# GestaltCogTeam/STEP

Hardware: AMD Instinct MI355X
Metric: training windows/sec on PEMS04, horizon-12 MAE parity, 1/2/4/8 MI355X (higher is better)
Workload: dtype f16 (TSFormer Q/K/weights) + bf16 (P, V, GraphWaveNet / graph-learner GEMMs) operands, f32 accumulate

## Files before the change

step_amd/csrc/common.h:

```cpp
#pragma once
#include "../../include/step_hip.h"
#include <hip/hip_runtime.h>
#include <stdint.h>
#include <stdio.h>
#include <string.h>

#define STEP_OK 0
#define STEP_ERR_ARG 1
#define STEP_ERR_HIP 2

void step_set_error(const char* fmt, ...);
int step_raise_lds_once(const void* kernel, int bytes, const char* what);

#define STEP_REQUIRE(cond, ...)                 \
    do {                                        \
        if (!(cond)) {                          \
            step_set_error(__VA_ARGS__);        \
            return STEP_ERR_ARG;                \
        }                                       \
    } while (0)

#define STEP_LAUNCH_CHECK(name)                                                   \
    do {                                                                          \
        hipError_t e_ = hipGetLastError();                                        \
        if (e_ != hipSuccess) {                                                   \
            step_set_error("%s: launch failed: %s", name, hipGetErrorString(e_)); \
            return STEP_ERR_HIP;                                                  \
        }                                                                         \
    } while (0)

#define STEP_TRY(expr)                       \
    do {                                     \
        int rc_ = (expr);                    \
        if (rc_ != STEP_OK) return rc_;      \
    } while (0)

typedef __attribute__((ext_vector_type(16))) float f32x16;
typedef __attribute__((ext_vector_type(4))) float f32x4;
typedef __attribute__((ext_vector_type(8))) __bf16 bf16x8;
typedef __attribute__((ext_vector_type(4))) uint32_t u32x4;
typedef __attribute__((ext_vector_type(2))) uint32_t u32x2;

static inline int cdiv(long a, long b) { return (int)((a + b - 1) / b); }

__device__ __forceinline__ uint32_t f32_to_bf16_bits(float f) {
    uint32_t u = __float_as_uint(f);
    u += 0x7fffu + ((u >> 16) & 1u);
    return u >> 16;
}
__device__ __forceinline__ uint32_t pack_bf16x2(float lo, float hi) {
    return f32_to_bf16_bits(lo) | (f32_to_bf16_bits(hi) << 16);
}
__device__ __forceinline__ float bf16_bits_to_f32(uint32_t b) { return __uint_as_float(b << 16); }

typedef __attribute__((ext_vector_type(8))) float f32x8;
__device__ __forceinline__ bf16x8 pack8(const float* v) {
    f32x8 t;
#pragma unroll
    for (int j = 0; j < 8; ++j) t[j] = v[j];
    return __builtin_convertvector(t, bf16x8);
}

__device__ __forceinline__ float wave_sum(float v) {
#pragma unroll
    for (int o = 32; o > 0; o >>= 1) v += __shfl_xor(v, o, 64);
    return v;
}
__device__ __forceinline__ float wave_max(float v) {
#pragma unroll
    for (int o = 32; o > 0; o >>= 1) v = fmaxf(v, __shfl_xor(v, o, 64));
    return v;
}

#ifndef STEP_PHILOX_MUL64
#define STEP_PHILOX_MUL64 1
#endif
__device__ __forceinline__ void philox4x32(uint32_t c0, uint32_t c1, uint32_t c2, uint32_t c3,
                                           uint32_t k0, uint32_t k1, uint32_t out[4]) {
#pragma unroll
    for (int r = 0; r < 10; ++r) {
#if STEP_PHILOX_MUL64
        const uint64_t p0 = (uint64_t)0xD2511F53u * c0, p1 = (uint64_t)0xCD9E8D57u * c2;
        const uint32_t hi0 = (uint32_t)(p0 >> 32), lo0 = (uint32_t)p0, hi1 = (uint32_t)(p1 >> 32), lo1 = (uint32_t)p1;
#else
        uint32_t hi0 = __umulhi(0xD2511F53u, c0), lo0 = 0xD2511F53u * c0;
        uint32_t hi1 = __umulhi(0xCD9E8D57u, c2), lo1 = 0xCD9E8D57u * c2;
#endif
        uint32_t n0 = hi1 ^ c1 ^ k0, n1 = lo1, n2 = hi0 ^ c3 ^ k1, n3 = lo0;
        c0 = n0; c1 = n1; c2 = n2; c3 = n3;
        k0 += 0x9E3779B9u; k1 += 0xBB67AE85u;
    }
    out[0] = c0; out[1] = c1; out[2] = c2; out[3] = c3;
}
__device__ __forceinline__ float u32_to_unit(uint32_t x) { return (float)(x >> 8) * (1.0f / 16777216.0f); }

struct GemmColAffine { float cs, csh; const float* mvec; };
__device__ __forceinline__ GemmColAffine gemm_col_affine(const StepGemm& g, int gn) {
    GemmColAffine a = {1.f, 0.f, nullptr};
    if (g.c_nscale) { const int c = gn / g.c_nperiod; a.cs = g.c_nscale[c]; a.csh = g.c_nshift[c]; a.mvec = g.c_mvec; }
    return a;
}

__device__ __forceinline__ void gemm_store_tile(const f32x16& acc, float* col, int mb, int M, long ldc, float alpha, int accumulate,
                                                float bv, int relu, GemmColAffine ca = GemmColAffine{1.f, 0.f, nullptr}) {
    float val[16];
#pragma unroll
    for (int e = 0; e < 16; ++e) {
        const int gm = mb + (e & 3) + 8 * (e >> 2);
        val[e] = alpha * acc[e] * ca.cs;
        if (ca.mvec) val[e] += ca.csh * (gm < M ? ca.mvec[gm] : 0.f);
    }
    if (accumulate == 2) {
#pragma unroll
        for (int e = 0; e < 16; ++e) {
            const int gm = mb + (e & 3) + 8 * (e >> 2);
            if (gm < M) atomicAdd(col + (long)gm * ldc, val[e]);
        }
    } else if (accumulate == 1) {
        float old[16];
// ... 23 lines not shown
```

step_amd/csrc/dgl.hip:

```cpp
#include "common.h"
#include "step_internal.h"

namespace {

constexpr int KW = 10;
constexpr int EMB = 100;

template <int CI, int CO, int TPT>
__global__ __launch_bounds__(256) void conv_relu_fwd_kernel(const float* __restrict__ in, const float* __restrict__ w,
                                                            const float* __restrict__ b, const float* __restrict__ in_sc,
                                                            const float* __restrict__ in_sh, float* __restrict__ out,
                                                            float* __restrict__ partial, int Tin, int stat_limit) {
    __shared__ __attribute__((aligned(16))) float ws[CI * KW * CO];
    __shared__ float red[4][2 * CO];
    const int tid = threadIdx.x, n = blockIdx.y;
    const int Tout = Tin - (KW - 1);
    for (int e = tid; e < CI * KW * CO; e += 256) {
        int co = e % CO, k = (e / CO) % KW, ci = e / (CO * KW);
        ws[e] = w[(co * CI + ci) * KW + k];
    }
    __syncthreads();
    const int t0 = (blockIdx.x * 256 + tid) * TPT;
    float acc[CO][TPT];
#pragma unroll
// ... 412 lines not shown
                                                            const StepDynState* __restrict__ dyn) {
    if (dyn) { const uint64_t x = dyn->seed_xor; seed_lo ^= (uint32_t)x; seed_hi ^= (uint32_t)(x >> 32); }
    const long E = (long)N * N;
    const int b = blockIdx.y;
    for (long e = (long)blockIdx.x * 256 + threadIdx.x; e < E; e += (long)gridDim.x * 256) {
        const float zv = z[e];
        float u0, u1;
        if (u) {
            u0 = u[((long)b * E + e) * 2];
            u1 = u[((long)b * E + e) * 2 + 1];
        } else {
            uint32_t r[4];
            philox4x32((uint32_t)e, (uint32_t)(e >> 32), (uint32_t)b, 0x5EEDu, seed_lo, seed_hi, r);
            u0 = u32_to_unit(r[0]); u1 = u32_to_unit(r[1]);
        }
        const float g0 = -logf(-logf(u0 + 1e-10f) + 1e-10f);
        const float g1 = -logf(-logf(u1 + 1e-10f) + 1e-10f);
        const float a0 = (zv + g0 - g1) * inv_tau;
        const float ys = 1.f / (1.f + __expf(-a0));
        const int i = (int)(e / N), j = (int)(e % N);
        theta[(long)b * E + e] = 1.f / (1.f + __expf(-zv));
        y0[(long)b * E + e] = ys;
        adj[(long)b * E + e] = (i != j && a0 >= 0.f) ? 1.f : 0.f;
    }
}

__global__ __launch_bounds__(256) void edge_dz_kernel(const float* __restrict__ dtheta, const float* __restrict__ dadj,
                                                      const float* __restrict__ theta, const float* __restrict__ y0, int B, int N,
                                                      float inv_tau, float* __restrict__ dz) {
    const long E = (long)N * N;
    for (long e = (long)blockIdx.x * 256 + threadIdx.x; e < E; e += (long)gridDim.x * 256) {
        const int i = (int)(e / N), j = (int)(e % N);
        float s = 0.f;
        for (int b = 0; b < B; ++b) {
            const long o = (long)b * E + e;
            float th = theta[o];
            if (dtheta) s += dtheta[o] * th * (1.f - th);
            if (dadj && i != j) { float y = y0[o]; s += dadj[o] * y * (1.f - y) * inv_tau; }
        }
        dz[e] = s;
    }
}

__global__ __launch_bounds__(256) void edge_bwd_row_kernel(const float* __restrict__ dz, const float* __restrict__ sndT,
                                                           const float* __restrict__ rcv, const float* __restrict__ wcat, int N,
                                                           float* __restrict__ drcv, float* __restrict__ dwcat, float* __restrict__ dbcat) {
    extern __shared__ float sdz[];
    __shared__ float sr[EMB], sw[EMB], ra[EMB], rh[EMB];
    __shared__ float red[4];
    const int i = blockIdx.x, tid = threadIdx.x, lane = tid & 63, wave = tid >> 6;
    if (tid < EMB) { sr[tid] = rcv[(long)i * EMB + tid]; sw[tid] = wcat[tid] - wcat[EMB + tid]; }
    float tot = 0.f;
    for (int j = tid; j < N; j += 256) { const float d = dz[(long)i * N + j]; sdz[j] = d; tot += d; }
    tot = wave_sum(tot);
    if (lane == 0) red[wave] = tot;
    __syncthreads();
    constexpr int FB = 5;
    static_assert(EMB % (4 * FB) == 0, "feature rounds");
    for (int f0 = wave * FB; f0 < EMB; f0 += 4 * FB) {
        float a[FB], h[FB], rf[FB];
        const float* srow[FB];
#pragma unroll
        for (int u = 0; u < FB; ++u) { a[u] = 0.f; h[u] = 0.f; rf[u] = sr[f0 + u]; srow[u] = sndT + (long)(f0 + u) * N; }
        const bool vec = (N & 3) == 0 && ((((uintptr_t)sndT) | ((uintptr_t)sdz)) & 15) == 0;
        const int n4 = vec ? N : 0;
        for (int j = 4 * lane; j < n4; j += 256) {
            const float4 d4 = *(const float4*)(sdz + j);
            float4 s4[FB];
#pragma unroll
            for (int u = 0; u < FB; ++u) s4[u] = *(const float4*)(srow[u] + j);
#pragma unroll
            for (int u = 0; u < FB; ++u) {
                const float h0 = rf[u] + s4[u].x, h1 = rf[u] + s4[u].y, h2 = rf[u] + s4[u].z, h3 = rf[u] + s4[u].w;
                const float m0 = h0 > 0.f ? d4.x : 0.f, m1 = h1 > 0.f ? d4.y : 0.f, m2 = h2 > 0.f ? d4.z : 0.f, m3 = h3 > 0.f ? d4.w : 0.f;
                a[u] += (m0 + m1) + (m2 + m3);
                h[u] += (m0 * h0 + m1 * h1) + (m2 * h2 + m3 * h3);
            }
        }
        for (int j = n4 + lane; j < N; j += 64) {
            const float d = sdz[j];
            float sv[FB];
#pragma unroll
            for (int u = 0; u < FB; ++u) sv[u] = srow[u][j];
#pragma unroll
            for (int u = 0; u < FB; ++u) {
                const float hid = rf[u] + sv[u];
                const float m = hid > 0.f ? d : 0.f;
                a[u] += m; h[u] += m * hid;
            }
        }
#pragma unroll
        for (int o = 32; o > 0; o >>= 1)
#pragma unroll
            for (int u = 0; u < FB; ++u) { a[u] += __shfl_xor(a[u], o, 64); h[u] += __shfl_xor(h[u], o, 64); }
        if (lane == 0) {
#pragma unroll
            for (int u = 0; u < FB; ++u) { ra[f0 + u] = a[u]; rh[f0 + u] = h[u]; }
        }
    }
    __syncthreads();
    if (tid < EMB) {
        drcv[(long)i * EMB + tid] = ra[tid] * sw[tid];
        atomicAdd(&dwcat[tid], rh[tid]);
        atomicAdd(&dwcat[EMB + tid], -rh[tid]);
    }
    if (tid == 0) {
        const float s = red[0] + red[1] + red[2] + red[3];
        atomicAdd(&dbcat[0], s);
        atomicAdd(&dbcat[1], -s);
    }
}
template <int VJ>
__global__ __launch_bounds__(256) void edge_bwd_col_kernel(const float* __restrict__ dz, const float* __restrict__ sndT,
                                                           const float* __restrict__ rcv, const float* __restrict__ wcat, int N,
                                                           float* __restrict__ dsndT) {
    const int lane = threadIdx.x & 63, wave = threadIdx.x >> 6;
    const int j = (blockIdx.x * 64 + lane) * VJ;
    const int f = blockIdx.y * 4 + wave;
    if (j >= N || f >= EMB) return;
    const float wd = wcat[f] - wcat[EMB + f];
    if constexpr (VJ == 4) {
        const float4 s4 = *(const float4*)(sndT + (long)f * N + j);
        float a0 = 0.f, a1 = 0.f, a2 = 0.f, a3 = 0.f;
#pragma unroll 8
        for (int i = 0; i < N; ++i) {
            const float r = rcv[(long)i * EMB + f];
            const float4 d = *(const float4*)(dz + (long)i * N + j);
            a0 += r + s4.x > 0.f ? d.x : 0.f; a1 += r + s4.y > 0.f ? d.y : 0.f;
            a2 += r + s4.z > 0.f ? d.z : 0.f; a3 += r + s4.w > 0.f ? d.w : 0.f;
        }
        *(float4*)(dsndT + (long)f * N + j) = make_float4(a0 * wd, a1 * wd, a2 * wd, a3 * wd);
    } else {
        const float s = sndT[(long)f * N + j];
        float a = 0.f;
#pragma unroll 8
        for (int i = 0; i < N; ++i) {
            float hid = rcv[(long)i * EMB + f] + s;
            float d = dz[(long)i * N + j];
            a += hid > 0.f ? d : 0.f;
        }
        dsndT[(long)f * N + j] = a * wd;
    }
}

__global__ void colsum_kernel(const float* __restrict__ x, long rows, int cols, long ld, float* __restrict__ out) {
    __shared__ float red[4][64];
    const int c = blockIdx.x * 64 + (threadIdx.x & 63);
// ... 10 lines not shown

int step_colsum_launch(const float* x, long rows, int cols, long ld, float* out, hipStream_t st) {
    int chunks = (int)((rows + 255) / 256);
    if (chunks > 512) chunks = 512;
    if (chunks < 1) chunks = 1;
    colsum_kernel<<<dim3(cdiv(cols, 64), chunks), 256, 0, st>>>(x, rows, cols, ld, out);
    STEP_LAUNCH_CHECK("colsum");
    return STEP_OK;
}

constexpr int DGL_SMALL = 256 + 64 + 1344 + 100 * 32;

__global__ void bn2_fused_coef_kernel(const float* __restrict__ dots, const float* __restrict__ stat, const float* __restrict__ gamma,
                                      double count, float* __restrict__ dgamma, float* __restrict__ dbeta, float* __restrict__ coef) {
    constexpr int C = 16;
    const int c = threadIdx.x;
    if (c >= C) return;
    const float S1 = dots[2 * c + 1];
    const float S2 = stat[3 * C + c] * (dots[2 * c] - stat[2 * C + c] * S1);
    dgamma[c] += S2;
    dbeta[c] += S1;
    coef[c] = (float)(S1 / count);
    coef[C + c] = (float)(S2 / count);
    coef[2 * C + c] = gamma[c] * stat[3 * C + c];
}

__global__ __launch_bounds__(256) void fc_prep_kernel(const float* __restrict__ fc_w, const float* __restrict__ st2, uint4* __restrict__ wp,
                                                      float* __restrict__ shiftdot, int T2) {
    __shared__ float red[4];
    const int o = blockIdx.y, t = blockIdx.x * 256 + threadIdx.x, tid = threadIdx.x;
    float acc = 0.f;
    if (t < T2) {
        float v[16];
#pragma unroll
        for (int c = 0; c < 16; ++c) v[c] = fc_w[((long)o * 16 + c) * T2 + t];
#pragma unroll
        for (int c = 0; c < 16; ++c) { acc += v[c] * st2[16 + c]; v[c] *= st2[c]; }
        uint4* dst = wp + ((long)o * T2 + t) * 2;
        dst[0] = make_uint4(pack_bf16x2(v[0], v[1]), pack_bf16x2(v[2], v[3]), pack_bf16x2(v[4], v[5]), pack_bf16x2(v[6], v[7]));
        dst[1] = make_uint4(pack_bf16x2(v[8], v[9]), pack_bf16x2(v[10], v[11]), pack_bf16x2(v[12], v[13]), pack_bf16x2(v[14], v[15]));
    }
    acc = wave_sum(acc);
    if ((tid & 63) == 0) red[tid >> 6] = acc;
    __syncthreads();
    if (tid == 0) atomicAdd(&shiftdot[o], red[0] + red[1] + red[2] + red[3]);
}
__global__ void gpre_init_kernel(float* __restrict__ gpre, const float* __restrict__ shiftdot, long n) {
    const long i = (long)blockIdx.x * 256 + threadIdx.x;
    if (i < n) gpre[i] = shiftdot[i % EMB];
}
__global__ __launch_bounds__(256) void fc_unpermute_kernel(const float* __restrict__ graw, const float* __restrict__ fc_w,
                                                           const float* __restrict__ st2, const float* __restrict__ colsum,
                                                           float* __restrict__ dfc_w, float* __restrict__ dots_o, int T2, int overwrite) {
    __shared__ float red[4][32];
    const int o = blockIdx.y, t = blockIdx.x * 256 + threadIdx.x, tid = threadIdx.x;
    const float cso = colsum[o];
    float d[32];
#pragma unroll
    for (int i = 0; i < 32; ++i) d[i] = 0.f;
    if (t < T2) {
        const float4* src = (const float4*)(graw + ((long)o * T2 + t) * 16);
        const float4 g0 = src[0], g1 = src[1], g2 = src[2], g3 = src[3];
        const float g[16] = {g0.x, g0.y, g0.z, g0.w, g1.x, g1.y, g1.z, g1.w, g2.x, g2.y, g2.z, g2.w, g3.x, g3.y, g3.z, g3.w};
        float w[16], old[16];
#pragma unroll
        for (int c = 0; c < 16; ++c) { const long idx = ((long)o * 16 + c) * T2 + t; w[c] = fc_w[idx]; old[c] = overwrite ? 0.f : dfc_w[idx]; }
#pragma unroll
        for (int c = 0; c < 16; ++c) {
            dfc_w[((long)o * 16 + c) * T2 + t] = old[c] + st2[c] * g[c] + st2[16 + c] * cso;
            d[2 * c] = w[c] * g[c]; d[2 * c + 1] = w[c] * cso;
        }
    }
#pragma unroll
    for (int i = 0; i < 32; ++i) {
        const float v = wave_sum(d[i]);
        if ((tid & 63) == 0) red[tid >> 6][i] = v;
    }
    __syncthreads();
    if (tid < 32) atomicAdd(&dots_o[o * 32 + tid], red[0][tid] + red[1][tid] + red[2][tid] + red[3][tid]);
}
__global__ void dots_reduce_kernel(const float* __restrict__ dots_o, float* __restrict__ dots) {
    const int i = threadIdx.x;
    if (i >= 32) return;
    double a = 0.0;
    for (int o = 0; o < EMB; ++o) a += dots_o[o * 32 + i];
    dots[i] = (float)a;
}

static bool dgl_channels_last(const StepDglParams* p) {
    const char* e = getenv("STEP_DGL_F32_STORAGE");
    return p->gemm_bf16 && !(e && e[0] == '1');
}

static bool dgl_legacy_bn_backward() {
    const char* e = getenv("STEP_DGL_LEGACY_BN");
    return e && e[0] == '1';
}

extern "C" long step_dgl_global_saved_floats(int N, int T) {
    long T1 = T - 9, T2 = T - 18;
    return (long)N * 8 * T1 + (long)N * 16 * T2 + (long)N * EMB + 4 * 8 + 4 * 16 + 4 * EMB + (long)EMB * 16 * T2 + 128;
}
static long fc_splitk_ws_floats(int N, int T2) {
    const int splits = step_gemm_auto_splitk(N, EMB, 16 * T2, 1);
    return splits > 1 ? (long)splits * N * EMB + 4 : 0;
}
static long wraw_floats(long T2) {
    const long w = (long)EMB * 16 * T2, pack = dgl_conv2_pack_floats();
    return w > pack ? w : pack;
}
extern "C" long step_dgl_global_work_floats(int N, int T, int backward) {
    long T1 = T - 9, T2 = T - 18;
    long nb1 = (long)N * cdiv(T1, 1024), nb2 = (long)N * cdiv(T2, 1024);
    long part = (nb1 > nb2 ? nb1 : nb2) * 32 + 64;
    if (!backward) return part + dgl_conv2_pack_floats() + 64 + fc_splitk_ws_floats(N, (int)T2);
    return part + (long)N * 16 * T2 + (long)N * 8 * T1 + wraw_floats(T2) + 2L * N * EMB + DGL_SMALL + dgl_conv2_wgrad_scratch_floats(N, (int)T1);
}

static float* saved_wp(float* saved, int N, int T) {
    long T1 = T - 9, T2 = T - 18;
    return saved + (long)N * 8 * T1 + (long)N * 16 * T2 + (long)N * EMB + 4 * 8 + 4 * 16 + 4 * EMB;
}
static void carve_saved(float* saved, int N, int T, float** a1, float** a2, float** gpre, float** st1, float** st2, float** st3) {
    long T1 = T - 9, T2 = T - 18;
    *a1 = saved; saved += (long)N * 8 * T1;
    *a2 = saved; saved += (long)N * 16 * T2;
    *gpre = saved; saved += (long)N * EMB;
    *st1 = saved; saved += 4 * 8;
    *st2 = saved; saved += 4 * 16;
    *st3 = saved;
}

// ... 360 lines not shown
```

step_amd/csrc/dgl_conv_mfma.hip:

```cpp
#include "common.h"
#include "step_internal.h"

namespace {

constexpr int KW = 10, CI = 8, CO = 16, C1_ = 8;
constexpr int FW_TT = 1024;

__device__ __forceinline__ uint32_t cvt2(float a, float b) {
    uint32_t r;
    asm("v_cvt_pk_bf16_f32 %0, %1, %2" : "=v"(r) : "v"(a), "v"(b));
    return r;
}
__device__ __forceinline__ bf16x8 as_frag(uint4 v) { return __builtin_bit_cast(bf16x8, v); }

__global__ __launch_bounds__(256) void conv2_fwd_mfma_kernel(const float* __restrict__ a1, const float* __restrict__ w,
                                                             const float* __restrict__ b, const float* __restrict__ sc,
                                                             const float* __restrict__ sh, float* __restrict__ a2,
                                                             float* __restrict__ partial, int T1) {
    __shared__ uint4 xs[FW_TT + 16];
    __shared__ float red[4][2 * CO];
    const int tid = threadIdx.x, lane = tid & 63, wave = tid >> 6, n = blockIdx.y;
    const int T2 = T1 - (KW - 1), t0 = blockIdx.x * FW_TT;
    const int ln = lane & 15, q = lane >> 4;

// ... 315 lines not shown
#pragma unroll
            for (int co = 0; co < C1; ++co) {
                bsum[co] += v[co];
                zs[co][tid] = (uint16_t)(cvt2(v[co], 0.f) & 0xffffu);
            }
            const uint16_t ha = (uint16_t)(cvt2(xa, 0.f) & 0xffffu);
            x0[tid] = ha;
            if (tid > 0) x1[tid - 1] = ha;
            if (tid < 10) {
                const uint16_t hb = (uint16_t)(cvt2(xb, 0.f) & 0xffffu);
                x0[tid + 256] = hb;
                x1[tid + 255] = hb;
            }
        }
        __syncthreads();
        if (pass + 1 < WG_PASSES && tp + WG_SC < T1) fetch(tp + WG_SC);
#pragma unroll
        for (int u = 0; u < 2; ++u) {
            const int tb = 64 * wave + 32 * u + 8 * q;
            uint4 av = *(const uint4*)&zs[ln & 7][tb];
            if (ln >= C1) av = make_uint4(0u, 0u, 0u, 0u);
            const int kk = ln < KW ? ln : 0;
            const uint16_t* row = (kk & 1) ? x1 : x0;
            const uint32_t* p = (const uint32_t*)(row + tb + (kk & ~1));
            uint4 bv = make_uint4(p[0], p[1], p[2], p[3]);
            if (ln >= KW) bv = make_uint4(0u, 0u, 0u, 0u);
            acc = __builtin_amdgcn_mfma_f32_16x16x32_bf16(as_frag(av), as_frag(bv), acc, 0, 0, 0);
        }
    }
    __syncthreads();
    if (wave > 0) {
#pragma unroll
        for (int e = 0; e < 4; ++e) red[wave - 1][lane][e] = acc[e];
    }
#pragma unroll
    for (int co = 0; co < C1; ++co) {
        const float sm = wave_sum(bsum[co]);
        if (lane == 0) redb[wave][co] = sm;
    }
    __syncthreads();
    float* out = partial + ((long)blockIdx.y * gridDim.x + blockIdx.x) * W1_OUT;
    if (wave == 0 && q < 2 && ln < KW) {
#pragma unroll
        for (int e = 0; e < 4; ++e)
            out[(4 * q + e) * KW + ln] = acc[e] + red[0][lane][e] + red[1][lane][e] + red[2][lane][e];
    }
    if (tid < C1) out[C1 * KW + tid] = redb[0][tid] + redb[1][tid] + redb[2][tid] + redb[3][tid];
}


__device__ __forceinline__ float bf16lo(uint32_t w) { return __uint_as_float(w << 16); }
__device__ __forceinline__ float bf16hi(uint32_t w) { return __uint_as_float(w & 0xffff0000u); }

__global__ __launch_bounds__(256) void conv1_fwd_cl_kernel(const float* __restrict__ x, const float* __restrict__ w,
                                                           const float* __restrict__ b, uint4* __restrict__ a1h,
                                                           float* __restrict__ partial, int T, int stat_limit) {
    __shared__ float ws[KW][C1_];
    __shared__ float red[4][2 * C1_];
    __shared__ __attribute__((aligned(16))) float xs[1024 + 16];
    const int tid = threadIdx.x, n = blockIdx.y, T1 = T - (KW - 1);
    if (tid < KW * C1_) ws[tid / C1_][tid % C1_] = w[(tid % C1_) * KW + tid / C1_];
    {
        const int tb = blockIdx.x * 1024;
        const float* xr = x + (long)n * T + tb;
        for (int i = tid; i < 1024 + 16; i += 256) xs[i] = tb + i < T ? xr[i] : 0.f;
    }
    __syncthreads();
    const int t0 = (blockIdx.x * 256 + tid) * 4;
    float s1[C1_], s2[C1_];
#pragma unroll
    for (int c = 0; c < C1_; ++c) { s1[c] = 0.f; s2[c] = 0.f; }
    if (t0 < T1) {
        float xv[16];
#pragma unroll
        for (int q4 = 0; q4 < 4; ++q4) {
            const float4 v4 = *(const float4*)(xs + 4 * tid + 4 * q4);
            xv[4 * q4] = v4.x; xv[4 * q4 + 1] = v4.y; xv[4 * q4 + 2] = v4.z; xv[4 * q4 + 3] = v4.w;
        }
        float acc[4][C1_];
#pragma unroll
        for (int j = 0; j < 4; ++j)
#pragma unroll
            for (int c = 0; c < C1_; ++c) acc[j][c] = b[c];
#pragma unroll
        for (int k = 0; k < KW; ++k)
#pragma unroll
            for (int c = 0; c < C1_; ++c) {
                const float wv = ws[k][c];
#pragma unroll
                for (int j = 0; j < 4; ++j) acc[j][c] += wv * xv[k + j];
            }
#pragma unroll
        for (int j = 0; j < 4; ++j) {
            if (t0 + j >= T1) break;
            float v[C1_];
#pragma unroll
            for (int c = 0; c < C1_; ++c) {
                v[c] = fmaxf(acc[j][c], 0.f);
                if (t0 + j < stat_limit) { s1[c] += v[c]; s2[c] += v[c] * v[c]; }
            }
            a1h[(long)n * T1 + t0 + j] = make_uint4(cvt2(v[0], v[1]), cvt2(v[2], v[3]), cvt2(v[4], v[5]), cvt2(v[6], v[7]));
        }
    }
    const int lane = tid & 63, wave = tid >> 6;
#pragma unroll
    for (int c = 0; c < C1_; ++c) {
        const float a = wave_sum(s1[c]), q = wave_sum(s2[c]);
        if (lane == 0) { red[wave][c] = a; red[wave][C1_ + c] = q; }
    }
    __syncthreads();
    if (tid < 2 * C1_)
        partial[((long)blockIdx.y * gridDim.x + blockIdx.x) * (2 * C1_) + tid] = red[0][tid] + red[1][tid] + red[2][tid] + red[3][tid];
}

__global__ void conv2_pack_kernel(const float* __restrict__ w, const float* __restrict__ b, const float* __restrict__ sc,
                                  const float* __restrict__ sh, uint4* __restrict__ pack) {
    const int lane = threadIdx.x & 63, s = threadIdx.x >> 6, ln = lane & 15, q = lane >> 4;
    float v[8];
    if (s < 3) {
        const int kk = 4 * s + q;
#pragma unroll
        for (int ci = 0; ci < CI; ++ci) v[ci] = kk < KW ? w[(ln * CI + ci) * KW + kk] * sc[ci] : 0.f;
    } else {
        const int kk = 2 * (s - 3) + (q >> 1), c0 = 8 * (q & 1);
#pragma unroll
        for (int j = 0; j < 8; ++j) v[j] = ln < CI ? w[((c0 + j) * CI + ln) * KW + kk] * sc[ln] : 0.f;
    }
    pack[s * 64 + lane] = make_uint4(cvt2(v[0], v[1]), cvt2(v[2], v[3]), cvt2(v[4], v[5]), cvt2(v[6], v[7]));
    if (threadIdx.x < CO) {
        float a = b[threadIdx.x];
        for (int ci = 0; ci < CI; ++ci) {
            float ws = 0.f;
            for (int kk = 0; kk < KW; ++kk) ws += w[(threadIdx.x * CI + ci) * KW + kk];
            a += ws * sh[ci];
        }
        ((float*)(pack + 8 * 64))[threadIdx.x] = a;
    }
}

__global__ __launch_bounds__(256) void conv2_fwd_cl_kernel(const uint4* __restrict__ a1h, const uint4* __restrict__ pack,
                                                           uint2* __restrict__ a2h, float* __restrict__ partial, int T1) {
    __shared__ uint4 xs[FW_TT + 16];
    __shared__ float red[4][2 * CO];
    const int tid = threadIdx.x, lane = tid & 63, wave = tid >> 6, n = blockIdx.y;
    const int T2 = T1 - (KW - 1), t0 = blockIdx.x * FW_TT;
    const int ln = lane & 15, q = lane >> 4;
    for (int tt = tid; tt < FW_TT + 16; tt += 256) {
        const int t = t0 + tt;
        xs[tt] = t < T1 ? a1h[(long)n * T1 + t] : make_uint4(0u, 0u, 0u, 0u);
    }
    bf16x8 wf[3];
#pragma unroll
    for (int s = 0; s < 3; ++s) wf[s] = as_frag(pack[s * 64 + lane]);
    float bias[4];
#pragma unroll
    for (int e = 0; e < 4; ++e) bias[e] = ((const float*)(pack + 8 * 64))[4 * q + e];
    __syncthreads();
    float s1[4] = {0.f, 0.f, 0.f, 0.f}, s2[4] = {0.f, 0.f, 0.f, 0.f};
    for (int tile = wave; tile < FW_TT / 16; tile += 4) {
        const int tb = tile * 16;
        if (t0 + tb >= T2) break;
        f32x4 acc = {0.f, 0.f, 0.f, 0.f};
#pragma unroll
        for (int s = 0; s < 3; ++s) acc = __builtin_amdgcn_mfma_f32_16x16x32_bf16(wf[s], as_frag(xs[tb + ln + 4 * s + q]), acc, 0, 0, 0);
        const int t = t0 + tb + ln;
        if (t < T2) {
            float v[4];
#pragma unroll
            for (int e = 0; e < 4; ++e) { v[e] = fmaxf(acc[e] + bias[e], 0.f); s1[e] += v[e]; s2[e] += v[e] * v[e]; }
            a2h[((long)n * T2 + t) * 4 + q] = make_uint2(cvt2(v[0], v[1]), cvt2(v[2], v[3]));
        }
    }
#pragma unroll
    for (int e = 0; e < 4; ++e) {
#pragma unroll
        for (int o = 1; o < 16; o <<= 1) { s1[e] += __shfl_xor(s1[e], o, 64); s2[e] += __shfl_xor(s2[e], o, 64); }
        if (ln == 0) { red[wave][4 * q + e] = s1[e]; red[wave][CO + 4 * q + e] = s2[e]; }
    }
    __syncthreads();
    if (tid < 2 * CO)
        partial[((long)blockIdx.y * gridDim.x + blockIdx.x) * (2 * CO) + tid] = red[0][tid] + red[1][tid] + red[2][tid] + red[3][tid];
}

__global__ __launch_bounds__(256) void conv2_dgrad_cl_kernel(const uint4* __restrict__ dz2h, const uint4* __restrict__ pack,
                                                             uint2* __restrict__ dz1h, int T1,
                                                             const uint2* __restrict__ a1h, const float* __restrict__ coef,
                                                             const float* __restrict__ stat, int own) {
    __shared__ uint4 zs[FW_TT + 16][2];
    const int tid = threadIdx.x, lane = tid & 63, wave = tid >> 6, n = blockIdx.y;
    const int T2 = T1 - (KW - 1), t0 = blockIdx.x * FW_TT;
    const int ln = lane & 15, q = lane >> 4;
    constexpr int NT = FW_TT / 16 / 4;
    uint2 xall[NT];
    if (q < 2) {
#pragma unroll
        for (int i = 0; i < NT; ++i) {
            const int t = t0 + (wave + 4 * i) * 16 + ln;
            xall[i] = t < T1 ? a1h[((long)n * T1 + t) * 2 + q] : make_uint2(0u, 0u);
        }
    }
    for (int tt = tid; tt < FW_TT + 16; tt += 256) {
        const int t = t0 - (KW - 1) + tt;
        const bool ok = t >= 0 && t < T2;
        zs[tt][0] = ok ? dz2h[((long)n * T2 + t) * 2] : make_uint4(0u, 0u, 0u, 0u);
        zs[tt][1] = ok ? dz2h[((long)n * T2 + t) * 2 + 1] : make_uint4(0u, 0u, 0u, 0u);
    }
    bf16x8 wf[5];
#pragma unroll
    for (int s = 0; s < 5; ++s) wf[s] = as_frag(pack[(3 + s) * 64 + lane]);
    float km1[4] = {0.f, 0.f, 0.f, 0.f}, km2[4] = {0.f, 0.f, 0.f, 0.f}, mu[4] = {0.f, 0.f, 0.f, 0.f};
    if (q < 2) {
#pragma unroll
        for (int e = 0; e < 4; ++e) {
            const int c = 4 * q + e;
            km1[e] = coef[2 * CI + c] * coef[c]; km2[e] = coef[2 * CI + c] * coef[CI + c] * stat[3 * CI + c]; mu[e] = stat[2 * CI + c];
        }
    }
    __syncthreads();
#pragma unroll
    for (int i = 0; i < NT; ++i) {
        const int tb = (wave + 4 * i) * 16;
        if (t0 + tb < T1) {
            f32x4 acc = {0.f, 0.f, 0.f, 0.f};
#pragma unroll
            for (int s = 0; s < 5; ++s) {
                const int kk = 2 * s + (q >> 1);
                acc = __builtin_amdgcn_mfma_f32_16x16x32_bf16(wf[s], as_frag(zs[tb + ln + (KW - 1) - kk][q & 1]), acc, 0, 0, 0);
            }
            const int t = t0 + tb + ln;
            if (t < T1 && q < 2) {
                const float x[4] = {bf16lo(xall[i].x), bf16hi(xall[i].x), bf16lo(xall[i].y), bf16hi(xall[i].y)};
                float o[4];
#pragma unroll
                for (int e = 0; e < 4; ++e) o[e] = x[e] > 0.f ? acc[e] - (t < own ? km1[e] + (x[e] - mu[e]) * km2[e] : 0.f) : 0.f;
                dz1h[((long)n * T1 + t) * 2 + q] = make_uint2(cvt2(o[0], o[1]), cvt2(o[2], o[3]));
            }
        }
    }
}

__global__ __launch_bounds__(256) void conv2_wgrad_cl_kernel(const uint4* __restrict__ dz2h, const uint4* __restrict__ a1h,
                                                             float* __restrict__ partial, int T1) {
    constexpr int ZP = WG_SC + 8, XP = WG_SC + 16;
    __shared__ __attribute__((aligned(16))) uint16_t zs[CO][ZP];
    __shared__ __attribute__((aligned(16))) uint16_t x0[CI][XP], x1[CI][XP];
    __shared__ float red[3][5][64][4];
    __shared__ float redb[4][CO];
    const int tid = threadIdx.x, lane = tid & 63, wave = tid >> 6, n = blockIdx.y;
    const int T2 = T1 - (KW - 1), tbeg = blockIdx.x * (WG_SC * WG_PASSES);
    const int ln = lane & 15, q = lane >> 4;
    f32x4 acc[5];
#pragma unroll
    for (int j = 0; j < 5; ++j) acc[j] = f32x4{0.f, 0.f, 0.f, 0.f};
    float bsum[CO];
#pragma unroll
    for (int co = 0; co < CO; ++co) bsum[co] = 0.f;
    uint4 z0, z1, xa, xb;
    auto fetch = [&](int tp) {
// ... 8 lines not shown
    fetch(tbeg);
    for (int pass = 0; pass < WG_PASSES; ++pass) {
        const int tp = tbeg + pass * WG_SC;
        if (tp >= T2) break;
        __syncthreads();
        {
            const uint32_t zw[8] = {z0.x, z0.y, z0.z, z0.w, z1.x, z1.y, z1.z, z1.w};
#pragma unroll
            for (int p = 0; p < 8; ++p) {
                bsum[2 * p] += bf16lo(zw[p]); bsum[2 * p + 1] += bf16hi(zw[p]);
                zs[2 * p][tid] = (uint16_t)(zw[p] & 0xffffu); zs[2 * p + 1][tid] = (uint16_t)(zw[p] >> 16);
            }
            const uint32_t xw[4] = {xa.x, xa.y, xa.z, xa.w};
#pragma unroll
            for (int p = 0; p < 4; ++p) {
                const uint16_t lo = (uint16_t)(xw[p] & 0xffffu), hi = (uint16_t)(xw[p] >> 16);
                x0[2 * p][tid] = lo; x0[2 * p + 1][tid] = hi;
                if (tid > 0) { x1[2 * p][tid - 1] = lo; x1[2 * p + 1][tid - 1] = hi; }
            }
            if (tid < 10) {
                const uint32_t yw[4] = {xb.x, xb.y, xb.z, xb.w};
#pragma unroll
                for (int p = 0; p < 4; ++p) {
                    const uint16_t lo = (uint16_t)(yw[p] & 0xffffu), hi = (uint16_t)(yw[p] >> 16);
                    x0[2 * p][tid + 256] = lo; x0[2 * p + 1][tid + 256] = hi;
                    x1[2 * p][tid + 255] = lo; x1[2 * p + 1][tid + 255] = hi;
                }
            }
        }
        __syncthreads();
        if (pass + 1 < WG_PASSES && tp + WG_SC < T2) fetch(tp + WG_SC);
#pragma unroll
        for (int u = 0; u < 2; ++u) {
            const int tb = 64 * wave + 32 * u + 8 * q;
            const bf16x8 a = as_frag(*(const uint4*)&zs[ln][tb]);
#pragma unroll
            for (int j = 0; j < 5; ++j) {
                const int kk = 2 * j + (ln >> 3), ci = ln & 7;
                const uint16_t* row = (kk & 1) ? &x1[ci][0] : &x0[ci][0];
                const uint32_t* p = (const uint32_t*)(row + tb + (kk & ~1));
                acc[j] = __builtin_amdgcn_mfma_f32_16x16x32_bf16(a, as_frag(make_uint4(p[0], p[1], p[2], p[3])), acc[j], 0, 0, 0);
            }
        }
    }
    __syncthreads();
    if (wave > 0) {
#pragma unroll
        for (int j = 0; j < 5; ++j)
#pragma unroll
            for (int e = 0; e < 4; ++e) red[wave - 1][j][lane][e] = acc[j][e];
    }
#pragma unroll
    for (int co = 0; co < CO; ++co) {
        const float sm = wave_sum(bsum[co]);
        if (lane == 0) redb[wave][co] = sm;
    }
    __syncthreads();
    float* out = partial + ((long)blockIdx.y * gridDim.x + blockIdx.x) * WG_OUT;
    if (wave == 0) {
#pragma unroll
        for (int j = 0; j < 5; ++j) {
            const int kk = 2 * j + (ln >> 3), ci = ln & 7;
#pragma unroll
            for (int e = 0; e < 4; ++e) out[((4 * q + e) * CI + ci) * KW + kk] = acc[j][e] + red[0][j][lane][e] + red[1][j][lane][e] + red[2][j][lane][e];
        }
    }
    if (tid < CO) out[CO * CI * KW + tid] = redb[0][tid] + redb[1][tid] + redb[2][tid] + redb[3][tid];
}

__global__ __launch_bounds__(256) void conv1_wgrad_cl_kernel(const uint4* __restrict__ dz1h, const float* __restrict__ x,
                                                             float* __restrict__ partial, int T) {
    constexpr int ZP = WG_SC + 8, XP = WG_SC + 16;
    __shared__ __attribute__((aligned(16))) uint16_t zs[C1][ZP];
    __shared__ __attribute__((aligned(16))) uint16_t x0[XP], x1[XP];
    __shared__ float red[3][64][4];
    __shared__ float redb[4][C1];
    const int tid = threadIdx.x, lane = tid & 63, wave = tid >> 6, n = blockIdx.y;
    const int T1 = T - (KW - 1), tbeg = blockIdx.x * (WG_SC * WG_PASSES);
    const int ln = lane & 15, q = lane >> 4;
    f32x4 acc = {0.f, 0.f, 0.f, 0.f};
    float bsum[C1];
#pragma unroll
    for (int co = 0; co < C1; ++co) bsum[co] = 0.f;
    uint4 z;
    float xa, xb;
    auto fetch = [&](int tp) {
        const int t = tp + tid;
        z = t < T1 ? dz1h[(long)n * T1 + t] : make_uint4(0u, 0u, 0u, 0u);
        xa = t < T ? x[(long)n * T + t] : 0.f;
        xb = (tid < 10 && t + 256 < T) ? x[(long)n * T + t + 256] : 0.f;
    };
    fetch(tbeg);
    for (int pass = 0; pass < WG_PASSES; ++pass) {
        const int tp = tbeg + pass * WG_SC;
        if (tp >= T1) break;
        __syncthreads();
        {
            const uint32_t zw[4] = {z.x, z.y, z.z, z.w};
#pragma unroll
            for (int p = 0; p < 4; ++p) {
                bsum[2 * p] += bf16lo(zw[p]); bsum[2 * p + 1] += bf16hi(zw[p]);
                zs[2 * p][tid] = (uint16_t)(zw[p] & 0xffffu); zs[2 * p + 1][tid] = (uint16_t)(zw[p] >> 16);
            }
            const uint16_t ha = (uint16_t)(cvt2(xa, 0.f) & 0xffffu);
            x0[tid] = ha;
            if (tid > 0) x1[tid - 1] = ha;
            if (tid < 10) {
                const uint16_t hb = (uint16_t)(cvt2(xb, 0.f) & 0xffffu);
                x0[tid + 256] = hb;
                x1[tid + 255] = hb;
            }
        }
        __syncthreads();
        if (pass + 1 < WG_PASSES && tp + WG_SC < T1) fetch(tp + WG_SC);
#pragma unroll
        for (int u = 0; u < 2; ++u) {
            const int tb = 64 * wave + 32 * u + 8 * q;
            uint4 av = *(const uint4*)&zs[ln & 7][tb];
            if (ln >= C1) av = make_uint4(0u, 0u, 0u, 0u);
            const int kk = ln < KW ? ln : 0;
            const uint16_t* row = (kk & 1) ? x1 : x0;
            const uint32_t* p = (const uint32_t*)(row + tb + (kk & ~1));
            uint4 bv = make_uint4(p[0], p[1], p[2], p[3]);
            if (ln >= KW) bv = make_uint4(0u, 0u, 0u, 0u);
            acc = __builtin_amdgcn_mfma_f32_16x16x32_bf16(as_frag(av), as_frag(bv), acc, 0, 0, 0);
        }
    }
    __syncthreads();
    if (wave > 0) {
#pragma unroll
        for (int e = 0; e < 4; ++e) red[wave - 1][lane][e] = acc[e];
    }
#pragma unroll
    for (int co = 0; co < C1; ++co) {
        const float sm = wave_sum(bsum[co]);
        if (lane == 0) redb[wave][co] = sm;
    }
    __syncthreads();
    float* out = partial + ((long)blockIdx.y * gridDim.x + blockIdx.x) * W1_OUT;
    if (wave == 0 && q < 2 && ln < KW) {
#pragma unroll
        for (int e = 0; e < 4; ++e) out[(4 * q + e) * KW + ln] = acc[e] + red[0][lane][e] + red[1][lane][e] + red[2][lane][e];
    }
    if (tid < C1) out[C1 * KW + tid] = redb[0][tid] + redb[1][tid] + redb[2][tid] + redb[3][tid];
}


}

static int wgrad_slices(long nrows) {
    long s = nrows / 256;
    return (int)(s < 16 ? 16 : (s > 128 ? 128 : s));
}

int dgl_conv2_fwd_mfma(const float* a1, const float* w, const float* b, const float* sc, const float* sh, float* a2, float* partial,
                       int N, int T1, int* nblk, hipStream_t st) {
    const int T2 = T1 - (KW - 1);
    dim3 grid(cdiv(T2, FW_TT), N);
    conv2_fwd_mfma_kernel<<<grid, 256, 0, st>>>(a1, w, b, sc, sh, a2, partial, T1);
    STEP_LAUNCH_CHECK("conv2_fwd_mfma");
    *nblk = grid.x * grid.y;
    return STEP_OK;
}

int dgl_conv2_dgrad_mfma(const float* dz, const float* w, float* din, int N, int T1, const float* bnx, const float* coef, const float* stat,
                         int own, hipStream_t st) {
    conv2_dgrad_mfma_kernel<<<dim3(cdiv(T1, FW_TT), N), 256, 0, st>>>(dz, w, din, T1, bnx, coef, stat, own);
    STEP_LAUNCH_CHECK("conv2_dgrad_mfma");
    return STEP_OK;
}

long dgl_conv2_wgrad_scratch_floats(int N, int T1) {
    const int T2 = T1 - (KW - 1);
    return (long)N * cdiv(T2, WG_SC * WG_PASSES) * WG_OUT;
}

int dgl_conv2_wgrad_mfma(const float* dz, const float* a1, const float* sc, const float* sh, float* scratch, float* dw, float* db, int N,
                         int T1, hipStream_t st) {
    const int T2 = T1 - (KW - 1);
    dim3 grid(cdiv(T2, WG_SC * WG_PASSES), N);
    conv2_wgrad_mfma_kernel<<<grid, 256, 0, st>>>(dz, a1, sc, sh, scratch, T1, 0);
    STEP_LAUNCH_CHECK("conv2_wgrad_mfma");
    conv_wgrad_reduce_kernel<<<dim3(cdiv(WG_OUT, 64), wgrad_slices(grid.x * grid.y)), 256, 0, st>>>(scratch, grid.x * grid.y, WG_OUT, CO * CI * KW, dw, db);
    STEP_LAUNCH_CHECK("conv2_wgrad_reduce");
    return STEP_OK;
}

int dgl_conv2_wgrad_xhat_mfma(const float* dz, const float* a1, const float* stat1, float* scratch, float* graw, int N, int T1,
                              hipStream_t st) {
    const int T2 = T1 - (KW - 1);
    dim3 grid(cdiv(T2, WG_SC * WG_PASSES), N);
    if (hipMemsetAsync(graw, 0, WG_OUT * sizeof(float), st) != hipSuccess) { step_set_error("memset failed"); return STEP_ERR_HIP; }
    conv2_wgrad_mfma_kernel<<<grid, 256, 0, st>>>(dz, a1, stat1, nullptr, scratch, T1, 1);
    STEP_LAUNCH_CHECK("conv2_wgrad_mfma(xhat)");
    conv_wgrad_reduce_kernel<<<dim3(cdiv(WG_OUT, 64), wgrad_slices(grid.x * grid.y)), 256, 0, st>>>(scratch, grid.x * grid.y, WG_OUT, CO * CI * KW, graw, graw + CO * CI * KW);
    STEP_LAUNCH_CHECK("conv2_wgrad_reduce");
    return STEP_OK;
}
int dgl_conv2_wgrad_finish(const float* graw, const float* w, const float* stat1, const float* gamma1, const float* beta1, double count,
                           float* dw, float* db, float* dgamma1, float* dbeta1, float* coef1, int raw, hipStream_t st) {
    conv2_wgrad_finish_kernel<<<1, 256, 0, st>>>(graw, w, stat1, gamma1, beta1, count, dw, db, dgamma1, dbeta1, coef1, raw);
    STEP_LAUNCH_CHECK("conv2_wgrad_finish");
    return STEP_OK;
}

int dgl_conv1_wgrad_mfma(const float* dz, const float* x, float* scratch, float* dw, float* db, int N, int T, hipStream_t st) {
    const int T1 = T - (KW - 1);
    dim3 grid(cdiv(T1, WG_SC * WG_PASSES), N);
    conv1_wgrad_mfma_kernel<<<grid, 256, 0, st>>>(dz, x, scratch, T);
    STEP_LAUNCH_CHECK("conv1_wgrad_mfma");
    conv_wgrad_reduce_kernel<<<dim3(cdiv(W1_OUT, 64), wgrad_slices(grid.x * grid.y)), 256, 0, st>>>(scratch, grid.x * grid.y, W1_OUT, C1 * KW, dw, db);
    STEP_LAUNCH_CHECK("conv1_wgrad_reduce");
    return STEP_OK;
}

int dgl_conv1_fwd_cl(const float* x, const float* w, const float* b, void* a1h, float* partial, int N, int T, int stat_limit, int* nblk,
                     hipStream_t st) {
    const int T1 = T - (KW - 1);
    dim3 grid(cdiv(T1, 1024), N);
    conv1_fwd_cl_kernel<<<grid, 256, 0, st>>>(x, w, b, (uint4*)a1h, partial, T, stat_limit);
    STEP_LAUNCH_CHECK("conv1_fwd_cl");
    *nblk = grid.x * grid.y;
    return STEP_OK;
}
long dgl_conv2_pack_floats() { return 8 * 64 * 4 + 16; }
int dgl_conv2_fwd_cl(const void* a1h, const float* w, const float* b, const float* sc, const float* sh, void* a2h, float* partial, int N,
                     int T1, int* nblk, float* pack, hipStream_t st) {
    const int T2 = T1 - (KW - 1);
    dim3 grid(cdiv(T2, FW_TT), N);
    conv2_pack_kernel<<<1, 512, 0, st>>>(w, b, sc, sh, (uint4*)pack);
    conv2_fwd_cl_kernel<<<grid, 256, 0, st>>>((const uint4*)a1h, (const uint4*)pack, (uint2*)a2h, partial, T1);
    STEP_LAUNCH_CHECK("conv2_fwd_cl");
    *nblk = grid.x * grid.y;
    return STEP_OK;
}
int dgl_conv2_dgrad_cl(const void* dz2h, const float* w, const float* sc, void* dz1h, int N, int T1, const void* a1h, const float* coef,
                       const float* stat, int own, float* pack, hipStream_t st) {
    conv2_pack_kernel<<<1, 512, 0, st>>>(w, w, sc, sc, (uint4*)pack);
    conv2_dgrad_cl_kernel<<<dim3(cdiv(T1, FW_TT), N), 256, 0, st>>>((const uint4*)dz2h, (const uint4*)pack, (uint2*)dz1h, T1, (const uint2*)a1h, coef, stat, own);
    STEP_LAUNCH_CHECK("conv2_dgrad_cl");
    return STEP_OK;
}
int dgl_conv2_wgrad_cl(const void* dz2h, const void* a1h, float* scratch, float* graw, int N, int T1, hipStream_t st) {
    const int T2 = T1 - (KW - 1);
    dim3 grid(cdiv(T2, WG_SC * WG_PASSES), N);
    if (hipMemsetAsync(graw, 0, WG_OUT * sizeof(float), st) != hipSuccess) { step_set_error("memset failed"); return STEP_ERR_HIP; }
    conv2_wgrad_cl_kernel<<<grid, 256, 0, st>>>((const uint4*)dz2h, (const uint4*)a1h, scratch, T1);
    STEP_LAUNCH_CHECK("conv2_wgrad_cl");
    conv_wgrad_reduce_kernel<<<dim3(cdiv(WG_OUT, 64), wgrad_slices(grid.x * grid.y)), 256, 0, st>>>(scratch, grid.x * grid.y, WG_OUT, CO * CI * KW, graw, graw + CO * CI * KW);
    STEP_LAUNCH_CHECK("conv2_wgrad_reduce");
    return STEP_OK;
}
int dgl_conv1_wgrad_cl(const void* dz1h, const float* x, float* scratch, float* dw, float* db, int N, int T, hipStream_t st) {
    const int T1 = T - (KW - 1);
    dim3 grid(cdiv(T1, WG_SC * WG_PASSES), N);
    conv1_wgrad_cl_kernel<<<grid, 256, 0, st>>>((const uint4*)dz1h, x, scratch, T);
    STEP_LAUNCH_CHECK("conv1_wgrad_cl");
    conv_wgrad_reduce_kernel<<<dim3(cdiv(W1_OUT, 64), wgrad_slices(grid.x * grid.y)), 256, 0, st>>>(scratch, grid.x * grid.y, W1_OUT, C1 * KW, dw, db);
    STEP_LAUNCH_CHECK("conv1_wgrad_reduce");
    return STEP_OK;
}
```

Baseline: 2366.

## Use DPP reductions and restructure conv1 forward with LDS-transposed coalesced stores

```diff
diff --git a/step_amd/csrc/common.h b/step_amd/csrc/common.h
--- a/step_amd/csrc/common.h
+++ b/step_amd/csrc/common.h
@@ -37,6 +37,7 @@
 
 typedef __attribute__((ext_vector_type(16))) float f32x16;
 typedef __attribute__((ext_vector_type(4))) float f32x4;
+typedef __attribute__((ext_vector_type(2))) float f32x2;
 typedef __attribute__((ext_vector_type(8))) __bf16 bf16x8;
 typedef __attribute__((ext_vector_type(4))) uint32_t u32x4;
 typedef __attribute__((ext_vector_type(2))) uint32_t u32x2;
@@ -65,6 +66,23 @@
 #pragma unroll
     for (int o = 32; o > 0; o >>= 1) v += __shfl_xor(v, o, 64);
     return v;
+}
+template <int CTRL, int ROW_MASK>
+__device__ __forceinline__ float dpp_add(float v) {
+    return v + __int_as_float(__builtin_amdgcn_update_dpp(0, __float_as_int(v), CTRL, ROW_MASK, 0xf, false));
+}
+__device__ __forceinline__ float row_sum_fast(float v) {
+    v = dpp_add<0x111, 0xf>(v);
+    v = dpp_add<0x112, 0xf>(v);
+    v = dpp_add<0x114, 0xf>(v);
+    v = dpp_add<0x118, 0xf>(v);
+    return v;
+}
+__device__ __forceinline__ float wave_sum_fast(float v) {
+    v = row_sum_fast(v);
+    v = dpp_add<0x142, 0xa>(v);
+    v = dpp_add<0x143, 0xc>(v);
+    return __int_as_float(__builtin_amdgcn_readlane(__float_as_int(v), 63));
 }
 __device__ __forceinline__ float wave_max(float v) {
 #pragma unroll
diff --git a/step_amd/csrc/dgl.hip b/step_amd/csrc/dgl.hip
--- a/step_amd/csrc/dgl.hip
+++ b/step_amd/csrc/dgl.hip
@@ -488,7 +488,7 @@
     if (tid < EMB) { sr[tid] = rcv[(long)i * EMB + tid]; sw[tid] = wcat[tid] - wcat[EMB + tid]; }
     float tot = 0.f;
     for (int j = tid; j < N; j += 256) { const float d = dz[(long)i * N + j]; sdz[j] = d; tot += d; }
-    tot = wave_sum(tot);
+    tot = wave_sum_fast(tot);
     if (lane == 0) red[wave] = tot;
     __syncthreads();
     constexpr int FB = 5;
@@ -526,9 +526,7 @@
             }
         }
 #pragma unroll
-        for (int o = 32; o > 0; o >>= 1)
-#pragma unroll
-            for (int u = 0; u < FB; ++u) { a[u] += __shfl_xor(a[u], o, 64); h[u] += __shfl_xor(h[u], o, 64); }
+        for (int u = 0; u < FB; ++u) { a[u] = wave_sum_fast(a[u]); h[u] = wave_sum_fast(h[u]); }
         if (lane == 0) {
 #pragma unroll
             for (int u = 0; u < FB; ++u) { ra[f0 + u] = a[u]; rh[f0 + u] = h[u]; }
@@ -645,8 +643,8 @@
 __global__ __launch_bounds__(256) void fc_unpermute_kernel(const float* __restrict__ graw, const float* __restrict__ fc_w,
                                                            const float* __restrict__ st2, const float* __restrict__ colsum,
                                                            float* __restrict__ dfc_w, float* __restrict__ dots_o, int T2, int overwrite) {
-    __shared__ float red[4][32];
-    const int o = blockIdx.y, t = blockIdx.x * 256 + threadIdx.x, tid = threadIdx.x;
+    __shared__ float red[16][32];
+    const int o = blockIdx.y, t = blockIdx.x * 256 + threadIdx.x, tid = threadIdx.x, lane = tid & 63, wave = tid >> 6;
     const float cso = colsum[o];
     float d[32];
 #pragma unroll
@@ -666,11 +664,16 @@
     }
 #pragma unroll
     for (int i = 0; i < 32; ++i) {
-        const float v = wave_sum(d[i]);
-        if ((tid & 63) == 0) red[tid >> 6][i] = v;
-    }
-    __syncthreads();
-    if (tid < 32) atomicAdd(&dots_o[o * 32 + tid], red[0][tid] + red[1][tid] + red[2][tid] + red[3][tid]);
+        const float v = row_sum_fast(d[i]);
+        if ((lane & 15) == 15) red[4 * wave + (lane >> 4)][i] = v;
+    }
+    __syncthreads();
+    if (tid < 32) {
+        float v = 0.f;
+#pragma unroll
+        for (int r = 0; r < 16; ++r) v += red[r][tid];
+        atomicAdd(&dots_o[o * 32 + tid], v);
+    }
 }
 __global__ void dots_reduce_kernel(const float* __restrict__ dots_o, float* __restrict__ dots) {
     const int i = threadIdx.x;
diff --git a/step_amd/csrc/dgl_conv_mfma.hip b/step_amd/csrc/dgl_conv_mfma.hip
--- a/step_amd/csrc/dgl_conv_mfma.hip
+++ b/step_amd/csrc/dgl_conv_mfma.hip
@@ -391,65 +391,104 @@
 __device__ __forceinline__ float bf16lo(uint32_t w) { return __uint_as_float(w << 16); }
 __device__ __forceinline__ float bf16hi(uint32_t w) { return __uint_as_float(w & 0xffff0000u); }
 
+constexpr int C1F_RUN = 8, C1F_HALF = 64 * C1F_RUN, C1F_WAVE = 2 * C1F_HALF, C1F_SPAN = 4 * C1F_WAVE;
+constexpr int C1F_ROW = C1F_RUN + 1;
+__device__ __forceinline__ int c1f_xi(int i) { return i + ((i >> 6) << 2); }
 __global__ __launch_bounds__(256) void conv1_fwd_cl_kernel(const float* __restrict__ x, const float* __restrict__ w,
                                                            const float* __restrict__ b, uint4* __restrict__ a1h,
                                                            float* __restrict__ partial, int T, int stat_limit) {
-    __shared__ float ws[KW][C1_];
-    __shared__ float red[4][2 * C1_];
-    __shared__ __attribute__((aligned(16))) float xs[1024 + 16];
-    const int tid = threadIdx.x, n = blockIdx.y, T1 = T - (KW - 1);
-    if (tid < KW * C1_) ws[tid / C1_][tid % C1_] = w[(tid % C1_) * KW + tid / C1_];
+    __shared__ uint4 buf[4 * 64 * C1F_ROW];
+    static_assert(sizeof(uint4) * 4 * 64 * C1F_ROW >= sizeof(float) * (C1F_SPAN + 16 + ((C1F_SPAN + 16) >> 6) * 4 + 4), "series window fits");
+    static_assert(sizeof(uint4) * 4 * 64 * C1F_ROW >= sizeof(float) * 2 * C1_ * 256, "statistics fit");
+    float* xs = (float*)buf;
+    const int tid = threadIdx.x, lane = tid & 63, wave = tid >> 6, n = blockIdx.y, T1 = T - (KW - 1);
+    const int tb = blockIdx.x * C1F_SPAN;
     {
-        const int tb = blockIdx.x * 1024;
+        constexpr int NLD = (C1F_SPAN + 16 + 255) / 256;
         const float* xr = x + (long)n * T + tb;
-        for (int i = tid; i < 1024 + 16; i += 256) xs[i] = tb + i < T ? xr[i] : 0.f;
-    }
-    __syncthreads();
-    const int t0 = (blockIdx.x * 256 + tid) * 4;
-    float s1[C1_], s2[C1_];
-#pragma unroll
-    for (int c = 0; c < C1_; ++c) { s1[c] = 0.f; s2[c] = 0.f; }
-    if (t0 < T1) {
-        float xv[16];
-#pragma unroll
-        for (int q4 = 0; q4 < 4; ++q4) {
-            const float4 v4 = *(const float4*)(xs + 4 * tid + 4 * q4);
-            xv[4 * q4] = v4.x; xv[4 * q4 + 1] = v4.y; xv[4 * q4 + 2] = v4.z; xv[4 * q4 + 3] = v4.w;
-        }
-        float acc[4][C1_];
-#pragma unroll
-        for (int j = 0; j < 4; ++j)
-#pragma unroll
-            for (int c = 0; c < C1_; ++c) acc[j][c] = b[c];
-#pragma unroll
-        for (int k = 0; k < KW; ++k)
-#pragma unroll
-            for (int c = 0; c < C1_; ++c) {
-                const float wv = ws[k][c];
-#pragma unroll
-                for (int j = 0; j < 4; ++j) acc[j][c] += wv * xv[k + j];
-            }
-#pragma unroll
-        for (int j = 0; j < 4; ++j) {
-            if (t0 + j >= T1) break;
-            float v[C1_];
-#pragma unroll
-            for (int c = 0; c < C1_; ++c) {
-                v[c] = fmaxf(acc[j][c], 0.f);
-                if (t0 + j < stat_limit) { s1[c] += v[c]; s2[c] += v[c] * v[c]; }
-            }
-            a1h[(long)n * T1 + t0 + j] = make_uint4(cvt2(v[0], v[1]), cvt2(v[2], v[3]), cvt2(v[4], v[5]), cvt2(v[6], v[7]));
-        }
-    }
-    const int lane = tid & 63, wave = tid >> 6;
-#pragma unroll
-    for (int c = 0; c < C1_; ++c) {
-        const float a = wave_sum(s1[c]), q = wave_sum(s2[c]);
-        if (lane == 0) { red[wave][c] = a; red[wave][C1_ + c] = q; }
-    }
-    __syncthreads();
-    if (tid < 2 * C1_)
-        partial[((long)blockIdx.y * gridDim.x + blockIdx.x) * (2 * C1_) + tid] = red[0][tid] + red[1][tid] + red[2][tid] + red[3][tid];
+        const int last = T - 1 - tb;
+        float r[NLD];
+#pragma unroll
+        for (int q = 0; q < NLD; ++q) r[q] = xr[min(min(tid + 256 * q, C1F_SPAN + 15), last)];
+#pragma unroll
+        for (int q = 0; q < NLD; ++q) {
+            const int i = tid + 256 * q;
+            if (i < C1F_SPAN + 16) xs[c1f_xi(i)] = i <= last ? r[q] : 0.f;
+        }
+    }
+    __syncthreads();
+    float xv[2][C1F_RUN + 12];
+#pragma unroll
+    for (int h = 0; h < 2; ++h)
+#pragma unroll
+        for (int q4 = 0; q4 < (C1F_RUN + 12) / 4; ++q4) {
+            const float4 v4 = *(const float4*)(xs + c1f_xi(wave * C1F_WAVE + h * C1F_HALF + C1F_RUN * lane + 4 * q4));
+            xv[h][4 * q4] = v4.x; xv[h][4 * q4 + 1] = v4.y; xv[h][4 * q4 + 2] = v4.z; xv[h][4 * q4 + 3] = v4.w;
+        }
+    __syncthreads();
+    f32x2 s1[C1_ / 2], s2[C1_ / 2];
+#pragma unroll
+    for (int cp = 0; cp < C1_ / 2; ++cp) { s1[cp] = f32x2{0.f, 0.f}; s2[cp] = f32x2{0.f, 0.f}; }
+    const int slim = stat_limit < T1 ? stat_limit : T1;
+    uint4* tr = buf + wave * (64 * C1F_ROW);
+#pragma unroll
+    for (int h = 0; h < 2; ++h) {
+        const int tw = tb + wave * C1F_WAVE + h * C1F_HALF;
+        const bool act = tw < T1;
+        if (act) {
+            const int t0 = tw + C1F_RUN * lane;
+            uint32_t o[C1F_RUN][C1_ / 2];
+#pragma unroll
+            for (int cp = 0; cp < C1_ / 2; ++cp) {
+                const int c0 = 2 * cp, c1 = c0 + 1;
+                f32x2 wv[KW];
+#pragma unroll
+                for (int k = 0; k < KW; ++k) wv[k] = f32x2{w[c0 * KW + k], w[c1 * KW + k]};
+                const f32x2 bv = {b[c0], b[c1]};
+#pragma unroll
+                for (int j = 0; j < C1F_RUN; ++j) {
+                    f32x2 a = bv;
+#pragma unroll
+                    for (int k = 0; k < KW; ++k) a = __builtin_elementwise_fma(wv[k], f32x2{xv[h][k + j], xv[h][k + j]}, a);
+                    const float v0 = fmaxf(a[0], 0.f), v1 = fmaxf(a[1], 0.f);
+                    const bool in = t0 + j < slim;
+                    const f32x2 vm = {in ? v0 : 0.f, in ? v1 : 0.f};
+                    s1[cp] += vm;
+                    s2[cp] = __builtin_elementwise_fma(vm, vm, s2[cp]);
+                    o[j][cp] = cvt2(v0, v1);
+                }
+            }
+#pragma unroll
+            for (int j = 0; j < C1F_RUN; ++j) tr[lane * C1F_ROW + j] = make_uint4(o[j][0], o[j][1], o[j][2], o[j][3]);
+        }
+        __syncthreads();
+        if (act) {
+            uint4 rows[C1F_RUN];
+#pragma unroll
+            for (int i = 0; i < C1F_RUN; ++i) {
+                const int s = i * 64 + lane;
+                rows[i] = tr[(s / C1F_RUN) * C1F_ROW + s % C1F_RUN];
+            }
+#pragma unroll
+            for (int i = 0; i < C1F_RUN; ++i) {
+                const int s = i * 64 + lane;
+                if (tw + s < T1) a1h[(long)n * T1 + tw + s] = rows[i];
+            }
+        }
+        __syncthreads();
+    }
+    float* red = (float*)buf;
+#pragma unroll
+    for (int c = 0; c < C1_; ++c) { red[c * 256 + tid] = s1[c >> 1][c & 1]; red[(C1_ + c) * 256 + tid] = s2[c >> 1][c & 1]; }
+    __syncthreads();
+    float* prow = partial + ((long)blockIdx.y * gridDim.x + blockIdx.x) * (2 * C1_);
+#pragma unroll
+    for (int u = 0; u < 4; ++u) {
+        const int v = 4 * wave + u;
+        const float* r = red + v * 256 + lane;
+        const float tot = wave_sum_fast((r[0] + r[64]) + (r[128] + r[192]));
+        if (lane == 0) prow[v] = tot;
+    }
 }
 
 __global__ void conv2_pack_kernel(const float* __restrict__ w, const float* __restrict__ b, const float* __restrict__ sc,
@@ -484,9 +523,16 @@
     const int tid = threadIdx.x, lane = tid & 63, wave = tid >> 6, n = blockIdx.y;
     const int T2 = T1 - (KW - 1), t0 = blockIdx.x * FW_TT;
     const int ln = lane & 15, q = lane >> 4;
-    for (int tt = tid; tt < FW_TT + 16; tt += 256) {
-        const int t = t0 + tt;
-        xs[tt] = t < T1 ? a1h[(long)n * T1 + t] : make_uint4(0u, 0u, 0u, 0u);
+    {
+        constexpr int NLD = (FW_TT + 16 + 255) / 256;
+        uint4 r[NLD];
+#pragma unroll
+        for (int u = 0; u < NLD; ++u) r[u] = a1h[(long)n * T1 + min(t0 + min(tid + 256 * u, FW_TT + 15), T1 - 1)];
+#pragma unroll
+        for (int u = 0; u < NLD; ++u) {
+            const int tt = tid + 256 * u;
+            if (tt < FW_TT + 16) xs[tt] = t0 + tt < T1 ? r[u] : make_uint4(0u, 0u, 0u, 0u);
+        }
     }
     bf16x8 wf[3];
 #pragma unroll
@@ -512,9 +558,8 @@
     }
 #pragma unroll
     for (int e = 0; e < 4; ++e) {
-#pragma unroll
-        for (int o = 1; o < 16; o <<= 1) { s1[e] += __shfl_xor(s1[e], o, 64); s2[e] += __shfl_xor(s2[e], o, 64); }
-        if (ln == 0) { red[wave][4 * q + e] = s1[e]; red[wave][CO + 4 * q + e] = s2[e]; }
+        const float a = row_sum_fast(s1[e]), b2 = row_sum_fast(s2[e]);
+        if (ln == 15) { red[wave][4 * q + e] = a; red[wave][CO + 4 * q + e] = b2; }
     }
     __syncthreads();
     if (tid < 2 * CO)
@@ -538,11 +583,24 @@
             xall[i] = t < T1 ? a1h[((long)n * T1 + t) * 2 + q] : make_uint2(0u, 0u);
         }
     }
-    for (int tt = tid; tt < FW_TT + 16; tt += 256) {
-        const int t = t0 - (KW - 1) + tt;
-        const bool ok = t >= 0 && t < T2;
-        zs[tt][0] = ok ? dz2h[((long)n * T2 + t) * 2] : make_uint4(0u, 0u, 0u, 0u);
-        zs[tt][1] = ok ? dz2h[((long)n * T2 + t) * 2 + 1] : make_uint4(0u, 0u, 0u, 0u);
+    {
+        constexpr int NLD = (FW_TT + 16 + 255) / 256;
+        uint4 r0[NLD], r1[NLD];
+#pragma unroll
+        for (int u = 0; u < NLD; ++u) {
+            const int t = max(min(t0 - (KW - 1) + min(tid + 256 * u, FW_TT + 15), T2 - 1), 0);
+            r0[u] = dz2h[((long)n * T2 + t) * 2];
+            r1[u] = dz2h[((long)n * T2 + t) * 2 + 1];
+        }
+#pragma unroll
+        for (int u = 0; u < NLD; ++u) {
+            const int tt = tid + 256 * u, t = t0 - (KW - 1) + tt;
+            const bool ok = t >= 0 && t < T2;
+            if (tt < FW_TT + 16) {
+                zs[tt][0] = ok ? r0[u] : make_uint4(0u, 0u, 0u, 0u);
+                zs[tt][1] = ok ? r1[u] : make_uint4(0u, 0u, 0u, 0u);
+            }
+        }
     }
     bf16x8 wf[5];
 #pragma unroll
@@ -657,7 +715,7 @@
     }
 #pragma unroll
     for (int co = 0; co < CO; ++co) {
-        const float sm = wave_sum(bsum[co]);
+        const float sm = wave_sum_fast(bsum[co]);
         if (lane == 0) redb[wave][co] = sm;
     }
     __syncthreads();
@@ -738,7 +796,7 @@
     }
 #pragma unroll
     for (int co = 0; co < C1; ++co) {
-        const float sm = wave_sum(bsum[co]);
+        const float sm = wave_sum_fast(bsum[co]);
         if (lane == 0) redb[wave][co] = sm;
     }
     __syncthreads();
@@ -822,7 +880,7 @@
 int dgl_conv1_fwd_cl(const float* x, const float* w, const float* b, void* a1h, float* partial, int N, int T, int stat_limit, int* nblk,
                      hipStream_t st) {
     const int T1 = T - (KW - 1);
-    dim3 grid(cdiv(T1, 1024), N);
+    dim3 grid(cdiv(T1, C1F_SPAN), N);
     conv1_fwd_cl_kernel<<<grid, 256, 0, st>>>(x, w, b, (uint4*)a1h, partial, T, stat_limit);
     STEP_LAUNCH_CHECK("conv1_fwd_cl");
     *nblk = grid.x * grid.y;
```

Measured after the change: 2404 (median of 6 runs). 1.6% higher.
